# Jonas477/mixed-integer-optimal-control---algorithm-tools

Measured on AMD Instinct MI355X. Metric: bellman_TRM! subproblems/sec (nt=65536, 4096 levels, budget=256) + HBM GB/s, higher is better.
Workload: dtype f64; 1 GPU; C4: nt=65536, 4096 levels (8x8x8x8 product), B=256, p=1, 1 subproblem(s) per GPU per step; parallelism=dp1 (independent subproblems; one GPU, no collective)

## Files before the change

### mixed-integer-optimal-control---algorithm-tools_amd/csrc/mioc_sdt.hip

```cpp
#include <hip/hip_runtime.h>

#include <cstdint>

#include "mioc_internal.h"
#include "mioc_sdt_common.h"

namespace mioc {

constexpr int SD_STRAD_N = 32;
template <int M>
__host__ __device__ constexpr bool sd_strad() {
  return M == 4;
}

#if defined(MIOC_STAMPS) && !defined(MIOC_STAMPS_TL)
__device__ unsigned long long g_sdt_stamps[4096][16];
#define SD_STAMP(k)                                                                          \
  do {                                                                                       \
    if (threadIdx.x == 0) sh.stamp[k] = __builtin_amdgcn_s_memtime();                         \
  } while (0)
#define SD_RSTAMP(k)                                                                         \
  do {                                                                                       \
    if (threadIdx.x == 0) sh.stamp[k] = __builtin_amdgcn_s_memrealtime();                     \
  } while (0)
#define SD_FLUSH()                                                                           \
  do {                                                                                       \
    if (threadIdx.x == 0)                                                                    \
      for (int _q = 0; _q < 16; ++_q) g_sdt_stamps[blockIdx.x][_q] = sh.stamp[_q];           \
  } while (0)
#define SD_TL(k) \
  do {           \
  } while (0)
#define SD_TL_AT(gg, ii, ntt, k) \
  do {                           \
  } while (0)
#define SD_TL_FLUSH(gg) \
  do {                  \
  } while (0)
#elif defined(MIOC_STAMPS)
__device__ unsigned long long g_sdt_tl[4096][64][8];
__shared__ unsigned long long sd_tl_lds[64][8];
#define SD_TL_AT(gg, ii, ntt, k)                                                                          \
  do {                                                                                                    \
    if (threadIdx.x == 0 && (gg) < 4096 && (unsigned)((ii) - ((ntt) >> 1)) < 64u)                          \
      sd_tl_lds[(ii) - ((ntt) >> 1)][k] = __builtin_amdgcn_s_memrealtime();                                \
  } while (0)
#define SD_TL(k) SD_TL_AT(g, i, P.nt, k)
#define SD_TL_FLUSH(gg)                                                                                   \
  do {                                                                                                    \
    if (threadIdx.x == 0 && (gg) < 4096)                                                                  \
      for (int _j = 0; _j < 64; ++_j)                                                                     \
        for (int _q = 0; _q < 8; ++_q) g_sdt_tl[gg][_j][_q] = sd_tl_lds[_j][_q];                           \
  } while (0)
#define SD_STAMP(k) \
  do {              \
  } while (0)
#define SD_RSTAMP(k) \
  do {               \
  } while (0)
#define SD_FLUSH() \
  do {             \
  } while (0)
#else
#define SD_TL(k) \
  do {           \
  } while (0)
#define SD_TL_AT(gg, ii, ntt, k) \
  do {                           \
  } while (0)
#define SD_TL_FLUSH(gg) \
  do {                  \
  } while (0)
#define SD_STAMP(k) \
  do {              \
  } while (0)
#define SD_RSTAMP(k) \
  do {               \
  } while (0)
#define SD_FLUSH() \
  do {             \
  } while (0)
#endif


template <int M>
__device__ __forceinline__ int sd_p2(int tid, int q) {
  constexpr int L = 1 << (3 * M), T = L / 8;
  return 2 * (tid + T * q);
}
template <int M>
__device__ __forceinline__ int sd_seam_pos(int w, int o) {
  constexpr int L = 1 << (3 * M), T = L / 8;
  return 2 * T * (o >> 7) + 128 * w + (o & 127);
}
constexpr int kSdHeadPos = 0;


template <int M, bool COOP>
__device__ __forceinline__ void sd_scan(const uint16_t *list, int nl, const double *psi, const double *a,
                                        const int *base, double beta, uint16_t *UU, double *outnat, double *redv,
                                        int *redj) {
  constexpr int L = 1 << (3 * M), T = L / 8, NW = T / 64;
  const int tid = sd_tid(), lane = tid & 63, w = tid >> 6;
  auto target = [&](int r, int *xl) {
    double t1 = 0.0;
#pragma unroll
    for (int m = 0; m < M; ++m) {
      xl[m] = (r >> (3 * m)) & 7;
      t1 = t1 + a[m] * (double)(base[m] + xl[m]);
    }
    return t1;
  };
  auto wave_min = [&](double &bv, int &bj) {
#pragma unroll
    for (int off = 32; off > 0; off >>= 1) {
      const double ov = __shfl_xor(bv, off);
      const int oj = __shfl_xor(bj, off);
      if (oj >= 0 && (bj < 0 || ov < bv || (ov == bv && oj < bj))) {
        bv = ov;
        bj = oj;
      }
    }
  };
  if constexpr (COOP) {
    for (int e = 0; e < nl; ++e) {
      const int r = list[e];
      int xl[M];
      const double t1 = target(r, xl);
      const unsigned dpre = sd_l1(sd_bytes(tid), sd_bytes(r & ((1 << (3 * (M - 1))) - 1)));
      double bv = INFINITY;
      int bj = -1;
#pragma unroll
      for (int s = 0; s < 8; ++s) {
        const int j = tid + T * s;
        const double val = (t1 + beta * (double)(dpre + (unsigned)abs(s - xl[M - 1]))) + psi[j];
        if (val < bv) {
          bv = val;
          bj = j;
        }
      }
      wave_min(bv, bj);
      if (lane == 0) {
        redv[e * NW + w] = bv;
        redj[e * NW + w] = bj;
      }
    }
    sd_bar();
    if (tid < nl) {
      double bv = INFINITY;
      int bj = -1;
      for (int q = 0; q < NW; ++q) {
        const double ov = redv[tid * NW + q];
        const int oj = redj[tid * NW + q];
        if (oj >= 0 && (bj < 0 || ov < bv || (ov == bv && oj < bj))) {
          bv = ov;
          bj = oj;
        }
      }
      const int r = list[tid];
      if (bj >= 0) UU[r] = (uint16_t)bj;
      outnat[r] = bj >= 0 ? bv : INFINITY;
    }
  } else {
    for (int e = w; e < nl; e += NW) {
      const int r = list ? (int)list[e] : e;
      if (!list && !__builtin_isnan(outnat[r])) continue;
      int xl[M];
      const double t1 = target(r, xl);
      const unsigned pr = sd_bytes(r);
      double bv = INFINITY;
      int bj = -1;
      for (int t = 0; t < L / 64; ++t) {
        const int j = lane + 64 * t;
        const unsigned d = sd_l1(sd_bytes(j), pr);
        const double val = (t1 + beta * (double)d) + psi[j];
        if (val < bv) {
          bv = val;
          bj = j;
        }
      }
      wave_min(bv, bj);
      if (lane == 0) {
        if (bj >= 0) UU[r] = (uint16_t)bj;
        outnat[r] = bj >= 0 ? bv : INFINITY;
      }
    }
  }
}

template <bool SC1>
__device__ __forceinline__ double sd_load8(const double *base, int bytes, int e) {
  if constexpr (SC1) {
    const sd_u32x2 w = __builtin_amdgcn_raw_buffer_load_b64(sd_rsrc(base, bytes), e * 8, 0, 16);
    return __hiloint2double((int)w.y, (int)w.x);
  } else {
    return base[e];
  }
}
template <bool SC1>
__device__ __forceinline__ void sd_load_pair(const double *base, int bytes, int ea, int eb, double &va, double &vb) {
  if constexpr (SC1) {
    const sd_u32x4 t = __builtin_amdgcn_raw_buffer_load_b128(sd_rsrc(base, bytes), ea * 8, 0, 16);
    va = __hiloint2double((int)t.y, (int)t.x);
    vb = __hiloint2double((int)t.w, (int)t.z);
  } else {
    const double2 t = *reinterpret_cast<const double2 *>(base + ea);
    va = t.x;
    vb = t.y;
  }
  if (eb != ea + 1) vb = sd_load8<SC1>(base, bytes, eb);
}
template <bool SC1>
__device__ __forceinline__ void sd_store16(double *base, int bytes, int e, unsigned long long lo,
                                           unsigned long long hi) {
  if constexpr (SC1) {
    const sd_u32x4 d = {(unsigned)lo, (unsigned)(lo >> 32), (unsigned)hi, (unsigned)(hi >> 32)};
    __builtin_amdgcn_raw_buffer_store_b128(d, sd_rsrc(base, bytes), e * 8, 0, 16);
  } else {
    *reinterpret_cast<ulonglong2 *>(base + e) = make_ulonglong2(lo, hi);
  }
}

template <int NW>
struct SdtShared {
  double redv[SD_COOP * NW];
  int redj[SD_COOP * NW];
  double rmn[NW], rmx[NW];
  int rnv[NW];
  int nlist[2];
  int redo[2];
  int stop;
  unsigned long long stamp[16];
  int nsp;
  int spj[SD_SPARSE];
  double spv[SD_SPARSE];
  int cnt[4];
};

template <int M>
__host__ __device__ constexpr size_t sd_slot_offset() {
  return ((size_t)1 << (3 * M)) * (2 * sizeof(double) + sizeof(uint16_t)) + SD_LCAP * sizeof(uint16_t);
}
template <int M>
__host__ __device__ constexpr size_t sd_dfuo_stride() {
  return (2 * M + 2) * sizeof(double);
}
template <int M>
__host__ __device__ constexpr size_t sd_strad_offset() {
  return sd_slot_offset<M>() + 2 * ((size_t)1 << (3 * M)) * sizeof(uint32_t);
}
template <int M>
__host__ __device__ constexpr size_t sd_dfuo_offset() {
  return sd_strad_offset<M>() + 2 * 8 * SD_STRAD_N * sizeof(uint16_t);
}
template <int M>
__host__ __device__ constexpr size_t sd_out_offset() {
  return sd_dfuo_offset<M>() + ((sd_dfuo_stride<M>() * (((size_t)1 << (3 * M - 3)) / 64) + 255) & ~(size_t)255);
}
template <int M>
__host__ __device__ constexpr size_t sd_lds_total() {
  return sd_out_offset<M>() + ((size_t)1 << (3 * M)) * sizeof(double);
}


struct SdPerm {
  uint2 in[4], out[4];
  uint32_t hin, hout;
  int pin_h, pout_h;
};
template <int M>
__device__ __forceinline__ void sd_perm_load(SdPerm &pm, const uint32_t *__restrict__ perm_all, const ProblemDev &P,
                                             const PyrGeom &G, int k, int i) {
  constexpr int T = 1 << (3 * M - 3);
// ... 116 lines not shown
    }
  }
  sd_wave_stats(pmn, pmx);
  if (lane == 0) {
    sh.rmn[w] = pmn;
    sh.rmx[w] = pmx;
    sh.rnv[w] = nv;
  }
  return valid;
}

template <int M, bool PERSIST, class Hooks>
__device__ __forceinline__ int sdt_body(const ProblemDev &P, const LevelsDev &Lv, const PyrGeom &G, int k, int cp,
                                         int i, unsigned valid, const uint2 (&ein_in)[4], const uint32_t *pin,
                                         const uint32_t *pout,
                                         double *Sout, uint16_t *UU, SdtShared<(1 << (3 * M - 3)) / 64> &sh,
                                         unsigned char *sds, Hooks &h, const double *__restrict__ df_all,
                                         const double *__restrict__ uo_all, int par, unsigned smask = 0,
                                         int srank = -1) {
  constexpr int L = 1 << (3 * M), T = L / 8, NW = T / 64, Smax = 7 * M;
  double *psi = reinterpret_cast<double *>(sds);
  double *dtv = psi + L;
  uint16_t *uu = reinterpret_cast<uint16_t *>(dtv + L);
  double *outv = reinterpret_cast<double *>(sds + sd_out_offset<M>());
  uint16_t *list = uu + L;
  const int tid = sd_tid(), lane = tid & 63;
  const double beta = Lv.beta;
  const double *dfi = PERSIST ? reinterpret_cast<const double *>(sds + sd_dfuo_offset<M>()) + (2 * M + 2) * (threadIdx.x >> 6)
                              : df_all + ((size_t)k * P.nt + i) * M;
  (void)uo_all;
  SD_RSTAMP(13);
  SD_STAMP(0);
  uint2 ein[4];
#pragma unroll
  for (int q = 0; q < 4; ++q) ein[q] = ein_in[q];
  double a[M];
  int lb[M];
#pragma unroll
  for (int m = 0; m < M; ++m) {
    a[m] = P.dt * dfi[m];
    lb[m] = G.base[m];
  }
  double pre = 0.0;
#pragma unroll
  for (int m = 0; m < M - 1; ++m) {
    const int nu = lb[m] + ((tid >> (3 * m)) & 7);
    pre = pre + a[m] * (double)nu;
  }

  const double inv = Lv.inv_beta;
  double qa = beta * (double)Smax;
#pragma unroll
  for (int m = 0; m < M; ++m) qa += fabs(a[m]) * (double)max(abs(lb[m]), abs(lb[m] + 7));
  double ref, base, g, tol;
  bool scale_ok;
  auto scale = [&](double lo, double hi) {
    const double rs = (hi - lo) * inv + (double)Smax;
    scale_ok = rs < 0x1p31;
    const int E = ilogb(fmin(rs, 0x1p31) * (1.0 + 0x1p-20) + 1.0) + 2;
    base = ldexp(1.0, E);
    g = ldexp(1.0, E - SD_GRID);
    tol = 3.0 * g + 0x1p-49 * (qa + fmax(fabs(lo), fabs(hi))) * inv;
    ref = lo;
  };
  auto stamp = [&](double x, int j) {
    const double y = (x - ref) * inv + base;
    return __hiloint2double(__double2hiint(y), (__double2loint(y) & ~SD_PAY) | (j << SD_CB));
  };
  auto stamp_inf = [&](double x, int j) {
    const double y = stamp(x, j);
    const unsigned m = x < INFINITY ? ~0u : 0u;
    return __hiloint2double((int)(((unsigned)__double2hiint(y) & m) | (0x7FF00000u & ~m)),
                            (int)((unsigned)__double2loint(y) & m));
  };
  double o[8];
  double dmin = INFINITY;
  auto pass = [&](int m, auto count_tag) {
    constexpr bool COUNT = decltype(count_tag)::value;
    int pos[8];
#pragma unroll
    for (int x = 0; x < 8; ++x) {
      pos[x] = sd_swz(sd_rank((int)threadIdx.x, m, x));
      o[x] = (COUNT && m == 0) ? psi[sd_rank((int)threadIdx.x, 0, x)] : dtv[pos[x]];
    }
    if (m == 0) {
#pragma unroll
      for (int x = 0; x < 8; ++x) o[x] = stamp_inf(o[x], sd_rank((int)threadIdx.x, 0, x));
    }
    if constexpr (COUNT) {
#pragma unroll
      for (int x = 1; x < 8; ++x) o[x] = sd_merge(o[x], o[x - 1] + 1.0, tol);
#pragma unroll
      for (int x = 6; x >= 0; --x) o[x] = sd_merge(o[x], o[x + 1] + 1.0, tol);
    } else {
      sd_sweeps(o, dmin);
    }
    if (m + 1 < M) {
#pragma unroll
      for (int x = 0; x < 8; ++x) dtv[pos[x]] = o[x];
    }
  };
  auto passes = [&](auto count_tag) {
#pragma unroll
    for (int m = 0; m < M; ++m) {
      pass(m, count_tag);
      if (m + 2 < M)
        sd_wave_sync();
      else if (m + 1 < M)
        sd_bar();
      SD_STAMP(3 + m);
    }
  };
  auto winners = [&](auto flag_tag) {
    constexpr bool FLAG = decltype(flag_tag)::value;
    unsigned listed = 0;
    int jx[8];
    double pv[8];
#pragma unroll
    for (int x = 0; x < 8; ++x) jx[x] = (__double2loint(o[x]) >> SD_CB) & ((1 << SD_RB) - 1);
#pragma unroll
    for (int x = 0; x < 8; ++x) pv[x] = psi[jx[x]];
#pragma unroll
    for (int x = 0; x < 8; ++x) {
      const int r = tid | (x << (3 * (M - 1))), j = jx[x];
      const bool fin = (valid >> x & 1) != 0;
      const bool flg = FLAG && (__double2loint(o[x]) & SD_CNT) != 0;
      const double dd = o[x] - stamp(pv[x], j);
      const double t1 = pre + a[M - 1] * (double)(lb[M - 1] + x);
      const double val = (t1 + beta * dd) + pv[x];
      if constexpr (FLAG) {
        listed |= (unsigned)(fin && flg) << x;
        uu[r] = (uint16_t)(fin && !flg ? j : 0xFFFF);
        outv[r] = fin ? (flg ? __longlong_as_double(0x7FF8000000000000ll) : val) : INFINITY;
      } else {
        uu[r] = (uint16_t)(fin ? j : 0xFFFF);
        outv[r] = fin ? val : INFINITY;
      }
    }
    return listed;
  };
  auto list_targets = [&](unsigned listed) {
    if (listed) {
      int e = atomicAdd(&sh.nlist[par], __popc(listed));
#pragma unroll
      for (int x = 0; x < 8; ++x)
        if (listed >> x & 1) {
          if (e < SD_LCAP) list[e] = (uint16_t)(tid | (x << (3 * (M - 1))));
          ++e;
        }
    }
  };
  int nf, nv;
  bool empty;
  {
    double pmn, pmx;
    sd_bar();
    if (tid == 0) sh.nlist[par ^ 1] = sh.redo[par ^ 1] = 0;
    h.early();
    {
      double mn[NW], mx[NW];
      int cn[NW];
#pragma unroll
      for (int q = 0; q < NW; ++q) {
        mn[q] = sh.rmn[q];
        mx[q] = sh.rmx[q];
        cn[q] = sh.rnv[q];
      }
      [[maybe_unused]] uint32_t e0 = 0, ef = 0;
      if constexpr (PERSIST) {
        static_assert(SD_FEW < L, "entry SD_FEW of the sphere order");
        e0 = pout[0];
        ef = pout[SD_FEW];
      }
      asm volatile("s_waitcnt lgkmcnt(0)" ::: "memory");
#pragma unroll
      for (int h = NW / 2; h >= 1; h >>= 1)
#pragma unroll
        for (int q = 0; q < h; ++q) {
          mn[q] = sd_min(mn[q], mn[q + h]);
          mx[q] = sd_max(mx[q], mx[q + h]);
          cn[q] += cn[q + h];
        }
      pmn = mn[0];
      pmx = mx[0];
      nf = cn[0] >> 16;
      nv = cn[0] & 0xFFFF;
      if constexpr (PERSIST) nv = (int)(e0 >> 16) > P.B - cp ? 0 : (int)(ef >> 16) > P.B - cp ? SD_FEW : SD_FEW + 1;
    }
    SD_STAMP(1);
    empty = __builtin_amdgcn_readfirstlane((int)(nv == 0 || !(pmn < INFINITY))) != 0;
    scale(pmn, pmx);
  }
  const bool sparse = !empty && nf <= SD_SPARSE;
  const bool direct = !empty && !sparse && (nv <= SD_FEW || !scale_ok || !(tol < base * 0x1p-20));

  int spj[SD_SPARSE];
  double spv[SD_SPARSE];
  if (sparse) {
    if (tid == 0) sh.nsp = 0;
    sd_bar();
#pragma unroll
    for (int q = 0; q < 4; ++q)
#pragma unroll
      for (int hh = 0; hh < 2; ++hh) {
        const int j = (int)((hh ? ein[q].y : ein[q].x) & 0xFFFFu);
        const double x = psi[j];
        if (x < INFINITY && !(sd_strad<M>() && hh && (smask >> (3 * q + 2) & 1))) {
          const int e = atomicAdd(&sh.nsp, 1);
          sh.spj[e] = j;
          sh.spv[e] = x;
        }
      }
    if (sd_strad<M>() && srank >= 0 && !(srank & 0x10000) && psi[srank & 0xFFFF] < INFINITY) {
      const int e = atomicAdd(&sh.nsp, 1);
      sh.spj[e] = srank & 0xFFFF;
      sh.spv[e] = psi[srank & 0xFFFF];
    }
    sd_bar();
#pragma unroll
    for (int e = 0; e < SD_SPARSE; ++e) {
      spj[e] = sh.spj[e];
      spv[e] = sh.spv[e];
    }
  }
  const bool transform = !direct && !empty && !sparse;
  h.go();
  if (transform) passes(std::false_type{});

  if (!empty) {
    unsigned listed = 0;
    if (!direct && !sparse) {
      winners(std::false_type{});
      if (__any(dmin <= tol) && lane == 0) sh.redo[par] = 1;
    } else {
#pragma unroll
      for (int x = 0; x < 8; ++x) {
        const int r = tid | (x << (3 * (M - 1)));
        double ov = INFINITY;
        int uj = 0xFFFF;
        if (direct) {
          listed |= valid & (1u << x);
        } else {
          if (valid >> x & 1) {
            const double t1 = pre + a[M - 1] * (double)(lb[M - 1] + x);
            double bv = INFINITY;
            int bj = 0xFFFF;
#pragma unroll
            for (int e = 0; e < SD_SPARSE; ++e) {
              if (e < nf) {
                const int j = spj[e];
                const unsigned d = sd_l1(sd_bytes(j), sd_bytes((unsigned)tid) | (unsigned)x << (8 * (M - 1)));
                const double val = (t1 + beta * (double)d) + spv[e];
                if (val < bv || (val == bv && j < bj)) {
                  bv = val;
                  bj = j;
                }
              }
            }
            ov = bv;
            uj = bj;
          }
        }
        uu[r] = (uint16_t)uj;
        outv[r] = (listed >> x & 1) ? __longlong_as_double(0x7FF8000000000000ll) : ov;
      }
    }
    list_targets(listed);
    auto scans = [&]() {
      const int nl = sh.nlist[par];
      if (nl) {
        if (nl <= SD_COOP)
          sd_scan<M, true>(list, nl, psi, a, lb, beta, uu, outv, sh.redv, sh.redj);
        else if (nl <= SD_LCAP)
          sd_scan<M, false>(list, nl, psi, a, lb, beta, uu, outv, sh.redv, sh.redj);
        else
          sd_scan<M, false>(nullptr, L, psi, a, lb, beta, uu, outv, sh.redv, sh.redj);
        if (tid == 0) sh.cnt[direct ? 1 : 0] += nl;
      }
      return nl;
    };
    const bool scan_first = PERSIST && direct;
    if (scan_first) {
      sd_bar();
      scans();
    }
    h.late_drain();
    sd_bar();
    h.publish();
    SD_STAMP(7);
    if (transform && sh.redo[par]) {
      passes(std::true_type{});
      list_targets(winners(std::true_type{}));
      sd_bar();
      if (tid == 0) ++sh.cnt[3];
    }
    if (!scan_first && scans()) sd_bar();
  }
  if (empty) {
#pragma unroll
    for (int x = 0; x < 8; ++x) outv[tid | (x << (3 * (M - 1)))] = INFINITY;
    reinterpret_cast<ulonglong2 *>(uu)[tid] = make_ulonglong2(~0ull, ~0ull);
    h.late_drain();
    sd_bar();
    h.publish();
  }
  SD_STAMP(8);
  uint2 eo[4];
#pragma unroll
  for (int q = 0; q < 4; ++q) eo[q] = *reinterpret_cast<const uint2 *>(pout + sd_p2<M>(tid, q));
  double go[8];
#pragma unroll
  for (int q = 0; q < 4; ++q) {
    go[2 * q] = outv[eo[q].x & 0xFFFFu];
    go[2 * q + 1] = outv[eo[q].y & 0xFFFFu];
  }
  const ulonglong2 ut = reinterpret_cast<const ulonglong2 *>(uu)[tid];
  h.tail(empty, outv);
#pragma unroll
  for (int q = 0; q < 4; ++q)
    h.store16(Sout, sd_p2<M>(tid, q), __double_as_longlong(go[2 * q]), __double_as_longlong(go[2 * q + 1]));
  *reinterpret_cast<ulonglong2 *>(UU + 8 * tid) = ut;
  SD_STAMP(9);
  SD_RSTAMP(14);
  return empty ? 1 : 0;
}

template <int M, bool SC1>
__device__ __forceinline__ void sd_issue_loads(double (&v)[8], const uint32_t *pin, int cp, const double *Sin,
                                               int sbytes, const double *r0) {
  constexpr int L = 1 << (3 * M);
  const int tid = threadIdx.x;
#pragma unroll
  for (int q = 0; q < 4; ++q) {
    const int p2 = sd_p2<M>(tid, q);
    const uint2 e = *reinterpret_cast<const uint2 *>(pin + p2);
    const int ra = cp - (int)(e.x >> 16), rb = cp - (int)(e.y >> 16);
    double va = INFINITY, vb = INFINITY;
    if (ra == rb && (ra >= 1 || (ra == 0 && !r0))) {
      sd_load_pair<SC1>(Sin, sbytes, ra * L + p2, ra * L + p2 + 1, va, vb);
    } else {
      if (ra >= 1 || (ra == 0 && !r0))
        va = sd_load8<SC1>(Sin, sbytes, ra * L + p2);
      else if (ra == 0)
        va = r0[p2];
      if (rb >= 1 || (rb == 0 && !r0))
        vb = sd_load8<SC1>(Sin, sbytes, rb * L + p2 + 1);
      else if (rb == 0)
        vb = r0[p2 + 1];
    }
    v[2 * q] = va;
    v[2 * q + 1] = vb;
  }
}

template <int M>
struct SdEdge {
  double a[M];
  int lb[M], uo[M];
  __device__ __forceinline__ SdEdge(const ProblemDev &P, const int *lb_g, int k, int i) {
    const double *dfi = P.df + ((size_t)k * P.nt + i) * M;
    const double *uoi = P.uold + ((size_t)k * P.nt + i) * M;
#pragma unroll
    for (int m = 0; m < M; ++m) {
      a[m] = P.dt * dfi[m];
      lb[m] = lb_g[m];
      uo[m] = (int)uoi[m];
    }
  }
  __device__ __forceinline__ double t1(int r) const {
    double t = 0.0;
#pragma unroll
    for (int m = 0; m < M; ++m) t = t + a[m] * (double)(lb[m] + ((r >> (3 * m)) & 7));
    return t;
  }
  __device__ __forceinline__ int bt(int r) const {
    int b = 0;
#pragma unroll
    for (int m = 0; m < M; ++m) b += abs(lb[m] + ((r >> (3 * m)) & 7) - uo[m]);
    return b;
  }
  static __device__ __forceinline__ unsigned dist(int r, int j) { return sd_l1(sd_bytes(r), sd_bytes(j)); }
};
__device__ __forceinline__ unsigned long long sd_pack4(const unsigned short *u) {
  return (unsigned long long)u[0] | (unsigned long long)u[1] << 16 | (unsigned long long)u[2] << 32 |
         (unsigned long long)u[3] << 48;
}

template <int M, bool PERSIST>
__device__ __forceinline__ void sdt_row0(const ProblemDev &P, const LevelsDev &Lv, int k, int i, const SdPerm &pm,
                                         const double *Sin_all, double *Sout_all, uint16_t *__restrict__ UU_all,
                                         size_t s_stride, size_t uu_stride_k, const int *lb_g, int32_t *loaded,
                                         int token) {
  constexpr int L = 1 << (3 * M);
  const int tid = threadIdx.x, B = P.B;
  const double beta = Lv.beta;
  const double *Sin = Sin_all + (size_t)k * s_stride;
  double *S0 = Sout_all + (size_t)k * s_stride;
  uint16_t *U0 = UU_all + (size_t)k * uu_stride_k + (size_t)i * ((size_t)(B + 1) * L);
  const double psi0 = sd_load8<PERSIST>(Sin, (B + 1) * L * (int)sizeof(double), pm.pin_h);
  const SdEdge<M> E(P, lb_g, k, i);
  asm volatile("s_waitcnt vmcnt(0)" ::: "memory");
  __syncthreads();
  if (PERSIST && tid == 0) __hip_atomic_store(loaded, token, __ATOMIC_RELAXED, __HIP_MEMORY_SCOPE_AGENT);
  const int j0 = (int)(pm.hin & 0xFFFFu);
  const bool src0 = (pm.hin >> 16) == 0 && psi0 < INFINITY;
#pragma unroll
  for (int q = 0; q < 4; ++q) {
    double o[2];
#pragma unroll
    for (int h = 0; h < 2; ++h) {
      const uint32_t e = h ? pm.out[q].y : pm.out[q].x;
      const int r = (int)(e & 0xFFFFu);
      const double val = (E.t1(r) + beta * (double)SdEdge<M>::dist(r, j0)) + psi0;
      o[h] = src0 && (int)(e >> 16) <= B && val < INFINITY ? val : INFINITY;
    }
    sd_store16<PERSIST>(S0, L * 8, sd_p2<M>(tid, q), __double_as_longlong(o[0]), __double_as_longlong(o[1]));
  }
  unsigned short u0[8];
#pragma unroll
  for (int x = 0; x < 8; ++x) {
    const int r = 8 * tid + x;
    const double val = (E.t1(r) + beta * (double)SdEdge<M>::dist(r, j0)) + psi0;
    u0[x] = src0 && E.bt(r) <= B && val < INFINITY ? (unsigned short)j0 : (unsigned short)0xFFFF;
  }
  *reinterpret_cast<ulonglong2 *>(U0 + 8 * tid) = make_ulonglong2(sd_pack4(u0), sd_pack4(u0 + 4));
}

template <int M, bool PERSIST>
__device__ __forceinline__ void sdt_rowB(const ProblemDev &P, const LevelsDev &Lv, int k, int i, const SdPerm &pm,
                                         const double *Sin_all, double *Sout_all, uint16_t *__restrict__ UU_all,
                                         size_t s_stride, size_t uu_stride_k, const int *lb_g,
                                         int32_t *__restrict__ counters, SdtShared<(1 << (3 * M - 3)) / 64> &sh,
                                         int32_t *loaded, int token) {
  constexpr int L = 1 << (3 * M), T = L / 8, NW = T / 64;
  const int tid = threadIdx.x, lane = tid & 63, w = tid >> 6, B = P.B;
  const double beta = Lv.beta;
  const double *Sin = Sin_all + (size_t)k * s_stride;
  double *SB = Sout_all + (size_t)k * s_stride + (size_t)B * L;
  uint16_t *UB = UU_all + (size_t)k * uu_stride_k + (size_t)i * ((size_t)(B + 1) * L) + (size_t)B * L;
  const int sbytes = (B + 1) * L * (int)sizeof(double);
  double v[8];
#pragma unroll
  for (int q = 0; q < 4; ++q) {
    const int p2 = sd_p2<M>(tid, q);
    const int ra = max(B - (int)(pm.in[q].x >> 16), 0), rb = max(B - (int)(pm.in[q].y >> 16), 0);
    sd_load_pair<PERSIST>(Sin, sbytes, ra * L + p2, rb * L + p2 + 1, v[2 * q], v[2 * q + 1]);
  }
  const SdEdge<M> E(P, lb_g, k, i);
  const int r0 = (int)(pm.hout & 0xFFFFu);
  const bool has0 = (pm.hout >> 16) == 0;
  const double t1b = E.t1(r0);
  double bv = INFINITY;
  int bj = -1;
#pragma unroll
  for (int q = 0; q < 4; ++q)
#pragma unroll
    for (int h = 0; h < 2; ++h) {
      const uint32_t e = h ? pm.in[q].y : pm.in[q].x;
      const int j = (int)(e & 0xFFFFu);
      const double x = (int)(e >> 16) > B ? INFINITY : v[2 * q + h];
      const double val = (t1b + beta * (double)SdEdge<M>::dist(r0, j)) + x;
      if (val < bv || (val == bv && bj >= 0 && j < bj)) {
        bv = val;
        bj = j;
      }
    }
#pragma unroll
  for (int off = 32; off > 0; off >>= 1) {
    const double ov = __shfl_xor(bv, off);
// ... 362 lines not shown
  int32_t *dk, *lk, *err;
  const uint32_t *pk;
  uint32_t *slot;
  __amdgpu_buffer_rsrc_t rs;
  const char *dfuo0;
  unsigned dfuo_st;
  const uint16_t *sk;
  uint16_t *sslot;
  unsigned char *sds;
  unsigned ldsb;
  __device__ __forceinline__ unsigned lds_slot(int step) const {
    return ldsb + (unsigned)sd_slot_offset<M>() + (unsigned)(step & 1) * (unsigned)(L * sizeof(uint32_t));
  }
  __device__ __forceinline__ unsigned lds_sslot(int step) const {
    return ldsb + (unsigned)sd_strad_offset<M>() + (unsigned)(step & 1) * (unsigned)(8 * SD_STRAD_N * sizeof(uint16_t));
  }
  SdtShared<(1 << (3 * M - 3)) / 64> *sh;
  int pcp, pi;
  int32_t *fp;
  int need, val;
  SdRaw raw;
  SdNext nx;
  const ProblemDev *Pp;
  const PyrGeom *Gp;
  unsigned valid_next;
  int whole;
  unsigned nbo;
  unsigned sob;
  bool stop_seen;

  __device__ __forceinline__ void early() {
    SD_TL_AT(g0, i, nt, 1);
    const int tid = sd_tid(), lane = tid & 63, s = lane < 32 ? lane + 1 : lane - 31;
    fp = lk + cp * SDT_FLAG_STRIDE;
    need = INT32_MIN;
    if (lane < 32) {
      const int r = ncp - s;
      if (has_next && s <= 7 * M && r >= 1 && r < lo && nt - 2 - ni > 0) {
        fp = dk + r * SDT_FLAG_STRIDE;
        need = nt - 2 - ni;
      }
    } else {
      const int r = cp + s;
      if (s <= 7 * M && r <= B && r >= hi && war > 0) {
        fp = lk + r * SDT_FLAG_STRIDE;
        need = war;
      }
    }
    val = sd_flag_poll(fp);
    if (tid == 0 && war > 0 && min(cp + 7 * M, B) >= max(cp + 1, hi)) ++sh->cnt[2];
  }
  __device__ __forceinline__ void go() {
    SD_TL_AT(g0, i, nt, 2);
    const int tid = sd_tid();
    bool ready = __all(val >= need);
    if (tid == 0) __hip_atomic_store(lk + cp * SDT_FLAG_STRIDE, nt - 1 - i, __ATOMIC_RELAXED, __HIP_MEMORY_SCOPE_AGENT);
    unsigned spins = 0;
    while (!ready) {
      if (sd_flag_poll(err) || ++spins > spin_limit) {
        if ((tid & 63) == 0) {
          __hip_atomic_store(err, 1, __ATOMIC_RELAXED, __HIP_MEMORY_SCOPE_AGENT);
          sh->stop = 1;
        }
        break;
      }
      __builtin_amdgcn_s_sleep(1);
      val = sd_flag_poll(fp);
      ready = __all(val >= need);
    }
    SD_TL_AT(g0, i, nt, 3);
    if (has_next) {
      const int same = *(const volatile __attribute__((address_space(3))) int32_t *)(
          sds + sd_dfuo_offset<M>() + (threadIdx.x >> 6) * sd_dfuo_stride<M>() + 16 * M);
      sd_read_next<M>(nx, slot + ((ni + 1) & 1) * L, sslot + ((ni + 1) & 1) * 8 * SD_STRAD_N);
      sd_issue_pipe<M>(raw, rs, nx, ncp, nbo, r0b + (unsigned)(ni + 1) * rowb, rowb);
      if (ni != i && !same) {
        sd_perm_dma_asm<M>(pk + (size_t)ni * L, lds_slot(ni));
        if constexpr (sd_strad<M>()) sd_strad_dma(sk + (size_t)ni * 8 * SD_STRAD_N, lds_sslot(ni));
      }
      sd_dfuo_dma<M>(dfuo0 + (size_t)((unsigned)ni * dfuo_st), ni >= 1, ldsb);
    }
    SD_TL_AT(g0, i, nt, 4);
  }
  __device__ __forceinline__ void late_drain() {
#ifdef SD_TL_DRAIN
    SD_TL_AT(g0, i, nt, 7);
#endif
    asm volatile("s_waitcnt vmcnt(0)" ::: "memory");
    SD_TL_AT(g0, i, nt, 5);
  }
  __device__ __forceinline__ void publish() {
    if (sd_tid() == 0 && pcp >= 0)
      __hip_atomic_store(dk + pcp * SDT_FLAG_STRIDE, nt - 1 - pi, __ATOMIC_RELAXED, __HIP_MEMORY_SCOPE_AGENT);
    stop_seen = sh->stop != 0;
    pcp = cp;
    pi = i;
  }
  __device__ __forceinline__ void store16(double *, int e, unsigned long long lo, unsigned long long hi) {
    sd_store16<true>(reg + sob / 8, L * 8, e, lo, hi);
  }
  double *reg;
  __device__ __forceinline__ void tail(bool empty, const double *outv) {
    if (!has_next) return;
    double v[8];
    sd_take<M>(v, raw);
    if (whole && (sd_tid() & 63) == 0 && (raw.e[0].x >> 16) == 0) v[0] = empty ? INFINITY : outv[raw.e[0].x & 0xFFFFu];
    const double xs = __hiloint2double((int)raw.sv.y, (int)raw.sv.x);
    valid_next = sdt_stats<M, true>(*Pp, *Gp, k, ncp, ni, v, raw.e, *sh, sds, nullptr, nullptr, raw.srank, xs);
  }
};

template <int M>
__global__ __launch_bounds__(1 << (3 * M - 3), 2) void k_sdt_run(ProblemDev P_arg, LevelsDev Lv_arg, PyrGeom G,
                                                              const uint32_t *__restrict__ perm_all, double *S_all,
                                                              size_t kstride, int NB, uint16_t *__restrict__ UU_all,
                                                              size_t uu_stride_k, int32_t *__restrict__ counters,
                                                              int32_t *flags, int nwg, unsigned spin_limit,
                                                              const double *__restrict__ df_all,
                                                              const double *__restrict__ uo_all,
                                                              const int32_t *__restrict__ same2,
                                                              const uint16_t *__restrict__ strad) {
  constexpr int L = 1 << (3 * M);
  extern __shared__ __attribute__((aligned(16))) unsigned char sds[];
  __shared__ SdtShared<(1 << (3 * M - 3)) / 64> sh;
  ProblemDev P = P_arg;
  LevelsDev Lv = Lv_arg;
  asm volatile("" : "+v"(P.dt), "+v"(Lv.beta), "+v"(Lv.inv_beta));
  asm volatile("" : "+v"(counters), "+v"(spin_limit));
  const int B = P.B, R = B + 1, nt = P.nt, tid = threadIdx.x;
  const int FR = R * SDT_FLAG_STRIDE;
  int32_t *done = flags, *loaded = flags + P.K * FR, *err = flags + 2 * P.K * FR;
  const int W = nwg / P.K;
  const int k = (int)blockIdx.x / W, wl = (int)blockIdx.x - k * W;
  if (k >= P.K) return;
  const int base = B / W, extra = B - base * W;
  const int lo = 1 + wl * base + max(0, wl - (W - extra)), hi = lo + base + (wl >= W - extra ? 1 : 0);
  __builtin_assume(lo < hi);
  uint32_t *slot = reinterpret_cast<uint32_t *>(sds + sd_slot_offset<M>());
  auto pslot = [&](int step) { return slot + (step & 1) * L; };
  double *reg = S_all + (size_t)k * kstride;
  SdPipe<M> h;
  h.lo = lo, h.hi = hi, h.B = B, h.war = 2 - NB, h.nt = nt, h.k = k, h.g0 = k * R + lo;
  h.spin_limit = spin_limit, h.rowb = (unsigned)L * 8u, h.bufb = (unsigned)R * h.rowb, h.r0b = (unsigned)NB * h.bufb;
  asm volatile("" : "+v"(err));
  h.dk = done + (size_t)k * FR, h.lk = loaded + (size_t)k * FR, h.err = err;
  h.pk = perm_all + (size_t)k * nt * L, h.slot = slot;
  h.rs = __builtin_amdgcn_make_buffer_rsrc(reg, 0, (int)(h.r0b + (unsigned)nt * h.rowb), 0x00020000);
  h.dfuo0 = sd_dfuo_src<M>(df_all + (size_t)k * nt * M, uo_all + (size_t)k * nt * M, same2 + (size_t)k * nt - 1);
  h.dfuo_st = sd_dfuo_step<M>();
  h.sds = sds, h.ldsb = sd_lds_addr(sds), h.sh = &sh;
  h.sk = strad ? strad + (size_t)k * nt * 8 * SD_STRAD_N : nullptr;
  h.sslot = reinterpret_cast<uint16_t *>(sds + sd_strad_offset<M>());
  asm volatile("" : "+v"(h.pk), "+v"(h.sk), "+v"(h.dk), "+v"(h.lk));
  h.reg = reg;
  h.pcp = -1, h.pi = 0;
  if (tid == 0) {
    sh.stop = 0;
    sh.cnt[0] = sh.cnt[1] = sh.cnt[2] = sh.cnt[3] = 0;
    sh.nlist[0] = sh.nlist[1] = sh.redo[0] = sh.redo[1] = 0;
  }
  sd_perm_dma_asm<M>(h.pk + (size_t)(nt - 1) * L, h.lds_slot(nt - 1));
  sd_perm_dma_asm<M>(h.pk + (size_t)(nt - 2) * L, h.lds_slot(nt - 2));
  if constexpr (sd_strad<M>()) {
    sd_strad_dma(h.sk + (size_t)(nt - 1) * 8 * SD_STRAD_N, h.lds_sslot(nt - 1));
    sd_strad_dma(h.sk + (size_t)(nt - 2) * 8 * SD_STRAD_N, h.lds_sslot(nt - 2));
  }
  sd_dfuo_dma<M>(h.dfuo0 + (size_t)((unsigned)(nt - 2) * h.dfuo_st), nt >= 3, h.ldsb);
  asm volatile("s_waitcnt vmcnt(0)" ::: "memory");
  sd_bar();
  sd_read_next<M>(h.nx, pslot(nt - 1), h.sslot + ((nt - 1) & 1) * 8 * SD_STRAD_N);
  sd_issue_pipe<M>(h.raw, h.rs, h.nx, lo, (unsigned)((nt - 1) % NB) * h.bufb, h.r0b + (unsigned)(nt - 1) * h.rowb,
                   h.rowb);
  __builtin_amdgcn_s_waitcnt(0x0F70);
  h.Pp = &P, h.Gp = &G, h.whole = hi - lo == 1;
  {
    double v[8];
    sd_take<M>(v, h.raw);
    const double xs = __hiloint2double((int)h.raw.sv.y, (int)h.raw.sv.x);
    h.valid_next = sdt_stats<M, true>(P, G, k, lo, nt - 2, v, h.raw.e, sh, sds, df_all, uo_all, h.raw.srank, xs);
  }
  int par = 0;
  bool stop = false;
  int bi = (nt - 2) % NB, bi1 = (nt - 1) % NB;
  uint16_t *uu_i = UU_all + (size_t)k * uu_stride_k + (size_t)(nt - 2) * ((size_t)R * L);
#pragma nounroll
  for (int i = nt - 2; i >= 0 && !stop; --i) {
#pragma nounroll
    for (int cp = lo; cp < hi && !stop; ++cp) {
      const bool last_row = cp + 1 == hi;
      h.cp = cp, h.i = i;
      h.ncp = last_row ? lo : cp + 1, h.ni = last_row ? i - 1 : i;
      h.has_next = h.ni >= 0;
      h.nbo = (unsigned)(last_row ? bi : bi1) * h.bufb;
      h.sob = (unsigned)bi * h.bufb + (unsigned)cp * h.rowb;
      const int g = cp == lo ? h.g0 : 1 << 30;
      (void)g;
      SD_TL(0);
      asm volatile("s_waitcnt vmcnt(5)" ::: "memory");
#ifndef SD_TL_DRAIN
      SD_TL(7);
#endif
      uint2 ein[4];
#pragma unroll
      for (int q = 0; q < 4; ++q) ein[q] = h.raw.e[q];
      sdt_body<M, true>(P, Lv, G, k, cp, i, h.valid_next, ein, pslot(i + 1), pslot(i), nullptr,
                        uu_i + (unsigned)cp * (unsigned)L, sh, sds, h, df_all, uo_all, par, h.raw.mask, h.raw.srank);
      par ^= 1;
      SD_TL(6);
      stop = h.stop_seen;
    }
    bi1 = bi;
    bi = bi == 0 ? NB - 1 : bi - 1;
    unsigned rows = (unsigned)R;
    asm volatile("" : "+s"(rows));
    uu_i = reinterpret_cast<uint16_t *>(reinterpret_cast<char *>(uu_i) - rows * (unsigned)(L * sizeof(uint16_t)));
    ++h.war;
  }
  if (sd_tid() == 0) {
    if (sh.cnt[0]) atomicAdd(&counters[0], sh.cnt[0]);
    if (sh.cnt[1]) atomicAdd(&counters[1], sh.cnt[1]);
    if (sh.cnt[2]) atomicAdd(&counters[4], sh.cnt[2]);
    if (sh.cnt[3]) atomicAdd(&counters[5], sh.cnt[3]);
  }
  SD_FLUSH();
  SD_TL_FLUSH(h.g0);
}

bool sdt_seam_lists(const PyrGeom &G) { return G.M == 4 && sd_strad<4>(); }

bool sdt_supported(const PyrGeom &G) {
  if (G.M != 3 && G.M != 4) return false;
  for (int m = 0; m < G.M; ++m)
    if (G.n[m] != 8) return false;
  return true;
}

hipError_t launch_sdt_prep(hipStream_t s, const ProblemDev &P, const LevelsDev &Lv, const PyrGeom &G,
                           const uint32_t *perm, double *V, double *S, size_t kstride, size_t r0off, uint16_t *UU,
                           size_t uu_stride_k) {
  if (!sdt_supported(G)) return hipErrorInvalidValue;
  if (G.M == 4) {
    hipLaunchKernelGGL(k_sdt_chain<4>, dim3(P.K), dim3(256), 0, s, P, G, Lv.beta, perm, V);
    hipLaunchKernelGGL(k_sdt_row0<4>, dim3(P.nt, P.K), dim3(512), 0, s, P, Lv, G, perm, (const double *)V, S, kstride,
                       r0off, UU, uu_stride_k);
  } else {
    hipLaunchKernelGGL(k_sdt_chain<3>, dim3(P.K), dim3(256), 0, s, P, G, Lv.beta, perm, V);
    hipLaunchKernelGGL(k_sdt_row0<3>, dim3(P.nt, P.K), dim3(64), 0, s, P, Lv, G, perm, (const double *)V, S, kstride,
                       r0off, UU, uu_stride_k);
  }
  return hipGetLastError();
}

hipError_t launch_sdt_run(hipStream_t s, const ProblemDev &P, const LevelsDev &Lv, const PyrGeom &G,
                          const uint32_t *perm, const int32_t *same2, const uint16_t *strad, double *S, size_t kstride,
                          int NB, uint16_t *UU,
                          size_t uu_stride_k, int32_t *counters, int32_t *flags, int nwg, unsigned spin_limit,
                          size_t lds) {
  if (!sdt_supported(G)) return hipErrorInvalidValue;
  void *args[] = {(void *)&P,     (void *)&Lv,       (void *)&G,         (void *)&perm,
                  (void *)&S,     (void *)&kstride,  (void *)&NB,        (void *)&UU,
                  (void *)&uu_stride_k, (void *)&counters, (void *)&flags, (void *)&nwg, (void *)&spin_limit,
                  (void *)&P.df,  (void *)&P.uold, (void *)&same2, (void *)&strad};
  if (G.M == 4) return hipLaunchKernel((const void *)k_sdt_run<4>, dim3(nwg), dim3(512), args, lds, s);
  return hipLaunchKernel((const void *)k_sdt_run<3>, dim3(nwg), dim3(64), args, lds, s);
}

int sdt_run_blocks_per_cu(const PyrGeom &G, size_t lds) {
  int n = 0;
  hipError_t e = G.M == 4 ? hipOccupancyMaxActiveBlocksPerMultiprocessor(&n, k_sdt_run<4>, 512, lds)
                          : hipOccupancyMaxActiveBlocksPerMultiprocessor(&n, k_sdt_run<3>, 64, lds);
  return e == hipSuccess ? n : 0;
}

hipError_t launch_sdt_step(hipStream_t s, const ProblemDev &P, const LevelsDev &Lv, const PyrGeom &G, int i,
                           const uint32_t *perm, const double *Sin, double *Sout, uint16_t *UU, size_t s_stride,
                           size_t uu_stride_k, int32_t *counters) {
  if (!sdt_supported(G)) return hipErrorInvalidValue;
  const dim3 grid(P.B >= 1 ? P.B : 1, P.K);
  const size_t lds = sdt_lds_bytes(G);
  if (G.M == 4)
    hipLaunchKernelGGL(k_sdt_step<4>, grid, dim3(512), lds, s, P, Lv, G, i, perm, Sin, Sout, UU, s_stride,
                       uu_stride_k, counters);
  else
    hipLaunchKernelGGL(k_sdt_step<3>, grid, dim3(64), lds, s, P, Lv, G, i, perm, Sin, Sout, UU, s_stride,
                       uu_stride_k, counters);
  return hipGetLastError();
}

#if defined(MIOC_STAMPS) && defined(MIOC_STAMPS_TL)
extern "C" int32_t mioc_debug_sdt_timeline(unsigned long long *out, int64_t nrows) {
  return hipMemcpyFromSymbol(out, HIP_SYMBOL(g_sdt_tl), (size_t)nrows * 64 * 8 * sizeof(unsigned long long)) ==
                 hipSuccess
             ? 0
             : -4;
}
#elif defined(MIOC_STAMPS)
extern "C" int32_t mioc_debug_sdt_stamps(unsigned long long *out, int64_t nblocks) {
  return hipMemcpyFromSymbol(out, HIP_SYMBOL(g_sdt_stamps), (size_t)nblocks * 16 * sizeof(unsigned long long)) ==
                 hipSuccess
             ? 0
             : -4;
}
#endif

}
```

### mixed-integer-optimal-control---algorithm-tools_amd/csrc/mioc_sdt_common.h

```cpp
#pragma once
#include <hip/hip_runtime.h>

#include <cstdint>

namespace mioc {

constexpr int SD_RB = 12;
constexpr int SD_CB = 6;
constexpr int SD_CNT = (1 << SD_CB) - 1;
constexpr int SD_PAY = (1 << (SD_CB + SD_RB)) - 1;
constexpr int SD_GRID = 52 - SD_CB - SD_RB;
constexpr int SD_COOP = 8;
constexpr int SD_FEW = 4;
constexpr int SD_SPARSE = 4;
constexpr int SD_LCAP = 512;

__device__ __forceinline__ double sd_min(double a, double b) {
  double r;
  asm("v_min_f64 %0, %1, %2" : "=v"(r) : "v"(a), "v"(b));
  return r;
}
__device__ __forceinline__ double sd_min_abs(double a, double b) {
  double r;
  asm("v_min_f64 %0, %1, |%2|" : "=v"(r) : "v"(a), "v"(b));
  return r;
}
__device__ __forceinline__ double sd_max(double a, double b) {
  double r;
  asm("v_max_f64 %0, %1, %2" : "=v"(r) : "v"(a), "v"(b));
  return r;
}

#define SD_MG(X, Y)                      \
  "v_add_f64 %9, %" #Y ", 1.0\n\t"       \
  "v_add_f64 %10, %" #X ", -%9\n\t"      \
  "v_min_f64 %" #X ", %" #X ", %9\n\t"   \
  "v_min_f64 %8, %8, |%10|\n\t"
__device__ __forceinline__ void sd_sweeps(double (&o)[8], double &dmin) {
  double t, d;
  asm(SD_MG(1, 0) SD_MG(2, 1) SD_MG(3, 2) SD_MG(4, 3) SD_MG(5, 4) SD_MG(6, 5) SD_MG(7, 6)
      SD_MG(6, 7) SD_MG(5, 6) SD_MG(4, 5) SD_MG(3, 4) SD_MG(2, 3) SD_MG(1, 2) SD_MG(0, 1)
      : "+v"(o[0]), "+v"(o[1]), "+v"(o[2]), "+v"(o[3]), "+v"(o[4]), "+v"(o[5]), "+v"(o[6]), "+v"(o[7]), "+v"(dmin),
        "=&v"(t), "=&v"(d));
}
#undef SD_MG

__device__ __forceinline__ int sd_tid() {
  int t = (int)threadIdx.x;
  asm volatile("" : "+v"(t));
  return t;
}

__device__ __forceinline__ void sd_bar() { asm volatile("s_waitcnt lgkmcnt(0)\n\ts_barrier" ::: "memory"); }

__device__ __forceinline__ double sd_merge(double a, double b, double tol) {
  const double m = sd_min(a, b);
  const bool close = fabs(a - b) <= tol;
  return __hiloint2double(__double2hiint(m), (int)((unsigned)__double2loint(m) + (close ? 1u : 0u)));
}

template <int CTRL>
__device__ __forceinline__ int sd_dpp_i(int x) {
  return __builtin_amdgcn_update_dpp(0, x, CTRL, 0xF, 0xF, true);
}
template <int CTRL>
__device__ __forceinline__ double sd_dpp_d(double x) {
  return __hiloint2double(sd_dpp_i<CTRL>(__double2hiint(x)), sd_dpp_i<CTRL>(__double2loint(x)));
}
__device__ __forceinline__ double sd_rdl(double x, int l) {
  return __hiloint2double(__builtin_amdgcn_readlane(__double2hiint(x), l), __builtin_amdgcn_readlane(__double2loint(x), l));
}
__device__ __forceinline__ void sd_minmax(double &mn, double &mx, double a, double b) {
  asm("v_min_f64 %0, %0, %2\n\tv_max_f64 %1, %1, %3" : "+v"(mn), "+v"(mx) : "v"(a), "v"(b));
}
__device__ __forceinline__ void sd_minmax_s(double &mn, double &mx, double a, double b) {
  asm("v_min_f64 %0, %2, %0\n\tv_max_f64 %1, %3, %1" : "+v"(mn), "+v"(mx) : "s"(a), "s"(b));
}
__device__ __forceinline__ void sd_wave_stats(double &mn, double &mx) {
#define SD_STEP(C) sd_minmax(mn, mx, sd_dpp_d<C>(mn), sd_dpp_d<C>(mx));
  SD_STEP(0xB1) SD_STEP(0x4E) SD_STEP(0x141) SD_STEP(0x140)
#undef SD_STEP
  const double n1 = sd_rdl(mn, 16), n2 = sd_rdl(mn, 32), n3 = sd_rdl(mn, 48);
  const double x1 = sd_rdl(mx, 16), x2 = sd_rdl(mx, 32), x3 = sd_rdl(mx, 48);
  sd_minmax_s(mn, mx, n1, x1);
  sd_minmax_s(mn, mx, n2, x2);
  sd_minmax_s(mn, mx, n3, x3);
}

__device__ __forceinline__ int sd_swz(int r) { return r ^ ((r >> 3) & 7) ^ (((r >> 6) & 3) << 3); }

__device__ __forceinline__ int sd_rank(int q, int m, int x) {
  const int lo = q & ((1 << (3 * m)) - 1);
  return lo | (x << (3 * m)) | ((q >> (3 * m)) << (3 * (m + 1)));
}

__device__ __forceinline__ unsigned sd_bytes(unsigned r) {
  return (r & 7u) | ((r & 0x38u) << 5) | ((r & 0x1C0u) << 10) | ((r & 0xE00u) << 15);
}
__device__ __forceinline__ unsigned sd_l1(unsigned pa, unsigned pb) { return __builtin_amdgcn_sad_u8(pa, pb, 0u); }

typedef unsigned int sd_u32x4 __attribute__((ext_vector_type(4)));
typedef unsigned int sd_u32x2 __attribute__((ext_vector_type(2)));
__device__ __forceinline__ __amdgpu_buffer_rsrc_t sd_rsrc(const double *base, int bytes) {
  return __builtin_amdgcn_make_buffer_rsrc(const_cast<double *>(base), 0, bytes, 0x00020000);
}

__device__ __forceinline__ void sd_wave_sync() { asm volatile("s_waitcnt lgkmcnt(0)" ::: "memory"); }

}
```

Before: 2.422 subproblems/s.

## Add single-reachable-target fast path and DPP wave argmin in Bellman step

```diff
diff --git a/mixed-integer-optimal-control---algorithm-tools_amd/csrc/mioc_sdt.hip b/mixed-integer-optimal-control---algorithm-tools_amd/csrc/mioc_sdt.hip
--- a/mixed-integer-optimal-control---algorithm-tools_amd/csrc/mioc_sdt.hip
+++ b/mixed-integer-optimal-control---algorithm-tools_amd/csrc/mioc_sdt.hip
@@ -112,13 +112,17 @@
     return t1;
   };
   auto wave_min = [&](double &bv, int &bj) {
-#pragma unroll
-    for (int off = 32; off > 0; off >>= 1) {
-      const double ov = __shfl_xor(bv, off);
-      const int oj = __shfl_xor(bj, off);
-      if (oj >= 0 && (bj < 0 || ov < bv || (ov == bv && oj < bj))) {
-        bv = ov;
-        bj = oj;
+    if constexpr (COOP) {
+      sd_wave_argmin(bv, bj);
+    } else {
+#pragma unroll
+      for (int off = 32; off > 0; off >>= 1) {
+        const double ov = __shfl_xor(bv, off);
+        const int oj = __shfl_xor(bj, off);
+        if (oj >= 0 && (bj < 0 || ov < bv || (ov == bv && oj < bj))) {
+          bv = ov;
+          bj = oj;
+        }
       }
     }
   };
@@ -541,6 +545,9 @@
   };
   int nf, nv;
   bool empty;
+  int onev = 0;
+  auto is_one = [&]() { return PERSIST && __builtin_amdgcn_readfirstlane(onev) != 0; };
+  [[maybe_unused]] uint32_t e0h = 0;
   {
     double pmn, pmx;
     sd_bar();
@@ -555,10 +562,11 @@
         mx[q] = sh.rmx[q];
         cn[q] = sh.rnv[q];
       }
-      [[maybe_unused]] uint32_t e0 = 0, ef = 0;
+      [[maybe_unused]] uint32_t e0 = 0, e1 = 0, ef = 0;
       if constexpr (PERSIST) {
         static_assert(SD_FEW < L, "entry SD_FEW of the sphere order");
         e0 = pout[0];
+        e1 = pout[1];
         ef = pout[SD_FEW];
       }
       asm volatile("s_waitcnt lgkmcnt(0)" ::: "memory");
@@ -574,11 +582,21 @@
       pmx = mx[0];
       nf = cn[0] >> 16;
       nv = cn[0] & 0xFFFF;
-      if constexpr (PERSIST) nv = (int)(e0 >> 16) > P.B - cp ? 0 : (int)(ef >> 16) > P.B - cp ? SD_FEW : SD_FEW + 1;
+      if constexpr (PERSIST) {
+        nv = (int)(e0 >> 16) > P.B - cp ? 0 : (int)(ef >> 16) > P.B - cp ? SD_FEW : SD_FEW + 1;
+        onev = nv != 0 && (int)(e1 >> 16) > P.B - cp && pmn < INFINITY && nf > SD_SPARSE;
+        asm volatile("" : "+v"(onev));
+        e0h = e0;
+      }
     }
     SD_STAMP(1);
     empty = __builtin_amdgcn_readfirstlane((int)(nv == 0 || !(pmn < INFINITY))) != 0;
-    scale(pmn, pmx);
+    if (is_one()) {
+      ref = base = g = tol = 0.0;
+      scale_ok = true;
+    } else {
+      scale(pmn, pmx);
+    }
   }
   const bool sparse = !empty && nf <= SD_SPARSE;
   const bool direct = !empty && !sparse && (nv <= SD_FEW || !scale_ok || !(tol < base * 0x1p-20));
@@ -618,7 +636,32 @@
 
   if (!empty) {
     unsigned listed = 0;
-    if (!direct && !sparse) {
+    if (is_one()) {
+      const int l0 = (int)(e0h & 0xFFFFu);
+      double t1 = 0.0;
+#pragma unroll
+      for (int m = 0; m < M; ++m) t1 = t1 + a[m] * (double)(lb[m] + ((l0 >> (3 * m)) & 7));
+      const int xt = (l0 >> (3 * (M - 1))) & 7;
+      const unsigned dpre = sd_l1(sd_bytes(tid), sd_bytes(l0 & ((1 << (3 * (M - 1))) - 1)));
+      double ps[8];
+#pragma unroll
+      for (int s = 0; s < 8; ++s) ps[s] = psi[tid + T * s];
+      double bv = INFINITY;
+      int bj = -1;
+#pragma unroll
+      for (int s = 0; s < 8; ++s) {
+        const double val = (t1 + beta * (double)(dpre + (unsigned)abs(s - xt))) + ps[s];
+        if (val < bv) {
+          bv = val;
+          bj = tid + T * s;
+        }
+      }
+      sd_wave_argmin(bv, bj);
+      if (lane == 0) {
+        sh.redv[tid >> 6] = bv;
+        sh.redj[tid >> 6] = bj;
+      }
+    } else if (!direct && !sparse) {
       winners(std::false_type{});
       if (__any(dmin <= tol) && lane == 0) sh.redo[par] = 1;
     } else {
@@ -668,7 +711,7 @@
       }
       return nl;
     };
-    const bool scan_first = PERSIST && direct;
+    const bool scan_first = PERSIST && direct && !is_one();
     if (scan_first) {
       sd_bar();
       scans();
@@ -683,7 +726,7 @@
       sd_bar();
       if (tid == 0) ++sh.cnt[3];
     }
-    if (!scan_first && scans()) sd_bar();
+    if (!scan_first && !is_one() && scans()) sd_bar();
   }
   if (empty) {
 #pragma unroll
@@ -694,16 +737,48 @@
     h.publish();
   }
   SD_STAMP(8);
-  uint2 eo[4];
-#pragma unroll
-  for (int q = 0; q < 4; ++q) eo[q] = *reinterpret_cast<const uint2 *>(pout + sd_p2<M>(tid, q));
   double go[8];
-#pragma unroll
-  for (int q = 0; q < 4; ++q) {
-    go[2 * q] = outv[eo[q].x & 0xFFFFu];
-    go[2 * q + 1] = outv[eo[q].y & 0xFFFFu];
-  }
-  const ulonglong2 ut = reinterpret_cast<const ulonglong2 *>(uu)[tid];
+  ulonglong2 ut;
+  if (is_one()) {
+    double pv[NW];
+    int pj[NW];
+#pragma unroll
+    for (int q = 0; q < NW; ++q) {
+      pv[q] = sh.redv[q];
+      pj[q] = sh.redj[q];
+    }
+    double bv = pv[0];
+    int bj = pj[0];
+#pragma unroll
+    for (int q = 1; q < NW; ++q)
+      if (pv[q] < bv || (pv[q] == bv && (unsigned)pj[q] < (unsigned)bj)) {
+        bv = pv[q];
+        bj = pj[q];
+      }
+    const int l0 = (int)(e0h & 0xFFFFu);
+    const bool fin = bj >= 0;
+#pragma unroll
+    for (int x = 0; x < 8; ++x) go[x] = INFINITY;
+    if (tid == 0) {
+      if (fin) go[0] = bv;
+      outv[l0] = go[0];
+      sh.cnt[1] += 1;
+    }
+    const bool mine = fin && tid == (l0 >> 3);
+    const int sft = 16 * (l0 & 3);
+    const unsigned long long cell = ~(0xFFFFull << sft) | ((unsigned long long)bj << sft);
+    ut = make_ulonglong2(mine && !(l0 & 4) ? cell : ~0ull, mine && (l0 & 4) ? cell : ~0ull);
+  } else {
+    uint2 eo[4];
+#pragma unroll
+    for (int q = 0; q < 4; ++q) eo[q] = *reinterpret_cast<const uint2 *>(pout + sd_p2<M>(tid, q));
+#pragma unroll
+    for (int q = 0; q < 4; ++q) {
+      go[2 * q] = outv[eo[q].x & 0xFFFFu];
+      go[2 * q + 1] = outv[eo[q].y & 0xFFFFu];
+    }
+    ut = reinterpret_cast<const ulonglong2 *>(uu)[tid];
+  }
   h.tail(empty, outv);
 #pragma unroll
   for (int q = 0; q < 4; ++q)
@@ -1372,6 +1447,7 @@
   h.sk = strad ? strad + (size_t)k * nt * 8 * SD_STRAD_N : nullptr;
   h.sslot = reinterpret_cast<uint16_t *>(sds + sd_strad_offset<M>());
   asm volatile("" : "+v"(h.pk), "+v"(h.sk), "+v"(h.dk), "+v"(h.lk));
+  asm volatile("" : "+v"(h.r0b), "+v"(h.war));
   h.reg = reg;
   h.pcp = -1, h.pi = 0;
   if (tid == 0) {
@@ -1403,6 +1479,7 @@
   bool stop = false;
   int bi = (nt - 2) % NB, bi1 = (nt - 1) % NB;
   uint16_t *uu_i = UU_all + (size_t)k * uu_stride_k + (size_t)(nt - 2) * ((size_t)R * L);
+  asm volatile("" : "+v"(uu_i));
 #pragma nounroll
   for (int i = nt - 2; i >= 0 && !stop; --i) {
 #pragma nounroll
diff --git a/mixed-integer-optimal-control---algorithm-tools_amd/csrc/mioc_sdt_common.h b/mixed-integer-optimal-control---algorithm-tools_amd/csrc/mioc_sdt_common.h
--- a/mixed-integer-optimal-control---algorithm-tools_amd/csrc/mioc_sdt_common.h
+++ b/mixed-integer-optimal-control---algorithm-tools_amd/csrc/mioc_sdt_common.h
@@ -87,6 +87,32 @@
   sd_minmax_s(mn, mx, n3, x3);
 }
 
+template <int CTRL, int ROWS>
+__device__ __forceinline__ int sd_dpp_rows_i(int x) {
+  return __builtin_amdgcn_update_dpp(x, x, CTRL, ROWS, 0xF, false);
+}
+template <int CTRL, int ROWS>
+__device__ __forceinline__ double sd_dpp_rows_d(double x) {
+  return __hiloint2double(sd_dpp_rows_i<CTRL, ROWS>(__double2hiint(x)), sd_dpp_rows_i<CTRL, ROWS>(__double2loint(x)));
+}
+__device__ __forceinline__ void sd_wave_argmin(double &bv, int &bj) {
+  double mn = bv, mx = bv;
+#define SD_STEP(C) sd_minmax(mn, mx, sd_dpp_d<C>(mn), sd_dpp_d<C>(mx));
+  SD_STEP(0xB1) SD_STEP(0x4E) SD_STEP(0x141) SD_STEP(0x140)
+#undef SD_STEP
+  sd_minmax(mn, mx, sd_dpp_rows_d<0x142, 0xA>(mn), sd_dpp_rows_d<0x142, 0xA>(mx));
+  sd_minmax(mn, mx, sd_dpp_rows_d<0x143, 0xC>(mn), sd_dpp_rows_d<0x143, 0xC>(mx));
+  const double wm = sd_rdl(mn, 63);
+  unsigned c = bv == wm ? (unsigned)bj : ~0u;
+#define SD_STEP(C) c = min(c, (unsigned)sd_dpp_i<C>((int)c));
+  SD_STEP(0xB1) SD_STEP(0x4E) SD_STEP(0x141) SD_STEP(0x140)
+#undef SD_STEP
+  c = min(c, (unsigned)sd_dpp_rows_i<0x142, 0xA>((int)c));
+  c = min(c, (unsigned)sd_dpp_rows_i<0x143, 0xC>((int)c));
+  bv = wm;
+  bj = __builtin_amdgcn_readlane((int)c, 63);
+}
+
 __device__ __forceinline__ int sd_swz(int r) { return r ^ ((r >> 3) & 7) ^ (((r >> 6) & 3) << 3); }
 
 __device__ __forceinline__ int sd_rank(int q, int m, int x) {
```

After: 2.487 subproblems/s (median of 6 runs). +2.7%, better.
